# deprekate/PHANOTATE

Hardware: AMD Instinct MI355X
Metric: Mbp/s annotated (whole node) on 50 kb synthetic phage contigs (higher is better)
Workload: dtype u8 bases / fp64 scores / int64 edge weights / int128 distances; 1 GPU; batch of 1000 synthetic 50000 bp phage contigs on one GPU, resident in HBM (BASELINE config 4); contigs_total=1000, contigs_rank0=1000, contig_length=50000

## Files before the change

### include/phx.h

```cpp
#ifndef PHX_H
#define PHX_H

#include <stddef.h>
#include <stdint.h>

#ifdef __cplusplus
extern "C" {
#endif

#define PHX_VERSION 410
#define PHX_MAX_CODONS 16

#define PHX_OK 0
#define PHX_E_ARG (-1)
#define PHX_E_NODEVICE (-10)
#define PHX_E_HIP (-11)
#define PHX_E_NOMEM (-12)
#define PHX_E_STATE (-13)
#define PHX_E_PARAM (-14)
#define PHX_E_IO (-15)

#define PHX_S_OK 0
#define PHX_S_BADLETTER (-2)
#define PHX_S_TOOSHORT (-3)
// ... 157 lines not shown
    int32_t called;
    int32_t bypass;
} phx_gene_drop;
int phx_drop_margins_flat(phx_ctx *ctx, phx_gene_drop *rec, int64_t cap, int64_t *offsets , int32_t *status , int64_t *total);
int phx_drop_ms(phx_ctx *ctx, float *ms );
int phx_drop_stats(phx_ctx *ctx, int64_t *out );

int phx_dump_text(phx_ctx *ctx, int32_t contig, char **text, int64_t *text_len);

int phx_solve(phx_ctx *ctx, int32_t V, int32_t E, const int32_t *src, const int32_t *dst, const uint64_t *w_limbs,
              int32_t n_limbs, int32_t source, int32_t target, int32_t *path_out, int32_t cap, int32_t *n_path,
              uint64_t *dist_limbs);

#define PHX_N_STAGES 14
int phx_set_profiling(phx_ctx *ctx, int on);
int phx_set_profiling_stages(phx_ctx *ctx, uint32_t stage_mask);
int phx_get_stage_ms(phx_ctx *ctx, float *ms , int32_t *launches , int reset);
const char *phx_stage_name(int k);
int64_t phx_plan_timeouts(phx_ctx *ctx);
int64_t phx_front_runs(phx_ctx *ctx);
int64_t phx_seg_runs(phx_ctx *ctx);
int64_t phx_seg_fallbacks(phx_ctx *ctx);
int phx_seg_stats(phx_ctx *ctx, int32_t i, int32_t *out, int32_t cap_records);
int phx_batch_sizes(phx_ctx *ctx, int64_t *L, int64_t *n_orf, int64_t *n_node, int64_t *n_edge);

int phx_synth_contig(uint64_t seed, int64_t L, char *out);
int phx_dec_eval(const char *op, const char *a, const char *b, int prec, char *out, int cap);
int phx_dd_eval(const char *op, double ah, double al, double bh, double bl, double *rh, double *rl);
int phx_dd_shortest(double x, uint64_t *digits, int32_t *exp10);

typedef struct phx_fasta phx_fasta;
int phx_fasta_read(const char *path, phx_fasta **out);
int32_t phx_fasta_count(const phx_fasta *f);
int phx_fasta_record(const phx_fasta *f, int32_t i, const char **name, const char **seq, int64_t *len);
int phx_fasta_arrays(const phx_fasta *f, const char **names, const char **seqs, int64_t *lens);
void phx_fasta_free(phx_fasta *f);
int phx_format_tabular(int32_t n, const char *const *names, const phx_gene *genes, const int64_t *offsets, const int32_t *status, char **text, int64_t *text_len);
int phx_format_margins(int32_t n, const char *const *names, const phx_orf_margin *rec, const int64_t *offsets, const int32_t *status, char **text, int64_t *text_len);
int phx_format_drops(int32_t n, const char *const *names, const phx_gene_drop *rec, const int64_t *offsets, const int32_t *status, char **text, int64_t *text_len);
void phx_free_text(char *text);

#ifdef __cplusplus
}
#endif
#endif
```

### phanotate_amd/_lib.py

```python
import ctypes as C
import os

import numpy as np

HERE = os.path.dirname(os.path.abspath(__file__))
SO = os.path.join(HERE, "libphx.so")
MAXC = 16
N_STAGES = 14


class Params(C.Structure):
    _fields_ = [
        ("minlen", C.c_int32),
        ("n_start", C.c_int32),
        ("start", (C.c_char * 4) * MAXC),
        ("start_w", C.c_double * MAXC),
        ("n_stop", C.c_int32),
        ("stop", (C.c_char * 4) * MAXC),
        ("start_w_text", (C.c_char * 32) * MAXC),
    ]


class Gene(C.Structure):
    _fields_ = [("left", C.c_int32), ("right", C.c_int32), ("strand", C.c_int32), ("frame", C.c_int32), ("score", C.c_double)]
# ... 100 lines not shown
        "phx_tap_nodes": (C.c_int, [vp, i32, vp]),
        "phx_tap_edges": (C.c_int, [vp, i32, vp]),
        "phx_tap_path": (C.c_int, [vp, i32, vp, i32, P(i32), vp, i32]),
        "phx_tap_dist": (C.c_int, [vp, i32, vp, i64]),
        "phx_tap_dist_target": (C.c_int, [vp, i32, vp, i64]),
        "phx_margins_flat": (C.c_int, [vp, vp, i64, vp, vp, P(i64)]),
        "phx_margins_ms": (C.c_int, [vp, P(C.c_float)]),
        "phx_format_margins": (C.c_int, [i32, vp, vp, vp, vp, P(vp), P(i64)]),
        "phx_drop_margins_flat": (C.c_int, [vp, vp, i64, vp, vp, P(i64)]),
        "phx_drop_ms": (C.c_int, [vp, P(C.c_float)]),
        "phx_drop_stats": (C.c_int, [vp, P(i64)]),
        "phx_format_drops": (C.c_int, [i32, vp, vp, vp, vp, P(vp), P(i64)]),
        "phx_solve": (C.c_int, [vp, i32, i32, vp, vp, vp, i32, i32, i32, vp, i32, P(i32), vp]),
        "phx_set_profiling": (C.c_int, [vp, C.c_int]),
        "phx_set_profiling_stages": (C.c_int, [vp, C.c_uint32]),
        "phx_get_stage_ms": (C.c_int, [vp, P(C.c_float), P(i32), C.c_int]),
        "phx_stage_name": (C.c_char_p, [C.c_int]),
        "phx_batch_sizes": (C.c_int, [vp, P(i64), P(i64), P(i64), P(i64)]),
        "phx_plan_timeouts": (C.c_int64, [vp]),
        "phx_front_runs": (C.c_int64, [vp]),
        "phx_seg_runs": (C.c_int64, [vp]),
        "phx_seg_fallbacks": (C.c_int64, [vp]),
        "phx_seg_stats": (C.c_int, [vp, C.c_int32, C.c_void_p, C.c_int32]),
        "phx_synth_contig": (C.c_int, [C.c_uint64, i64, C.c_char_p]),
        "phx_fasta_read": (C.c_int, [C.c_char_p, P(vp)]),
        "phx_fasta_count": (i32, [vp]),
        "phx_fasta_record": (C.c_int, [vp, i32, P(vp), P(vp), P(i64)]),
        "phx_fasta_arrays": (C.c_int, [vp, vp, vp, vp]),
        "phx_fasta_free": (None, [vp]),
        "phx_format_tabular": (C.c_int, [i32, vp, vp, vp, vp, P(vp), P(i64)]),
        "phx_free_text": (None, [vp]),
    }
    for name, (res, args) in sig.items():
        f = getattr(L, name)
        f.restype = res
        f.argtypes = args
    assert GENE_DT.itemsize == C.sizeof(Gene)
    assert MARGIN_DT.itemsize == 40
    assert DROP_DT.itemsize == 40
    _lib = L
    return L


EXPORTS = ["phx_version", "phx_device_count", "phx_strerror", "phx_last_error", "phx_default_params", "phx_params_from_flags", "phx_set_exact", "phx_pool_create", "phx_pool_destroy", "phx_pool_last_error", "phx_pool_annotate", "phx_dump_text", "phx_dec_eval", "phx_dd_eval", "phx_dd_shortest", "phx_create", "phx_create_ex", "phx_destroy",
           "phx_annotate", "phx_free_results", "phx_upload", "phx_attach", "phx_set_trnas", "phx_run", "phx_run_async", "phx_wait", "phx_download", "phx_download_flat", "phx_certified", "phx_tap_globals",
           "phx_tap_positions", "phx_tap_orfs", "phx_tap_nodes", "phx_tap_edges", "phx_tap_path", "phx_tap_dist", "phx_solve", "phx_set_profiling", "phx_set_profiling_stages",
           "phx_get_stage_ms", "phx_stage_name", "phx_batch_sizes", "phx_plan_timeouts", "phx_front_runs", "phx_seg_runs", "phx_seg_fallbacks", "phx_seg_stats", "phx_synth_contig", "phx_fasta_read", "phx_fasta_count",
           "phx_fasta_record", "phx_fasta_arrays", "phx_fasta_free", "phx_format_tabular", "phx_free_text",
           "phx_margins_flat", "phx_tap_dist_target", "phx_margins_ms", "phx_format_margins",
           "phx_drop_margins_flat", "phx_drop_ms", "phx_drop_stats", "phx_format_drops"]
```

### phanotate_amd/api.py

```python
import ctypes as C

import numpy as np

from . import _lib
from ._lib import PhxError


def make_params(start_codons="atg:0.85,gtg:0.10,ttg:0.05", stop_codons="tag,tga,taa", minlen=90):
    p = _lib.Params()
    rc = _lib.lib().phx_params_from_flags(start_codons.encode(), stop_codons.encode(), int(minlen), C.byref(p))
    if rc:
        raise ValueError("start / stop codons %r / %r, minlen %r: libphx takes codon:weight pairs and codons of exactly 3 letters out of acgt, "
                         "at most %d of each, minlen >= 6 (%s)" % (start_codons, stop_codons, minlen, _lib.MAXC, _lib.lib().phx_strerror(rc).decode()))
    p.start_codons_text = start_codons
    return p


def synth_contig(seed, L=50000):
    buf = C.create_string_buffer(int(L))
    rc = _lib.lib().phx_synth_contig(int(seed), int(L), buf)
    if rc:
        raise PhxError(rc, "phx_synth_contig")
    return buf.raw

# ... 352 lines not shown

    def stage_ms(self, reset=True):
        ms = (C.c_float * _lib.N_STAGES)()
        nl = (C.c_int32 * _lib.N_STAGES)()
        self._chk(self.L.phx_get_stage_ms(self.h, ms, nl, 1 if reset else 0), "phx_get_stage_ms")
        return {self.L.phx_stage_name(k).decode(): (float(ms[k]), int(nl[k])) for k in range(_lib.N_STAGES)}

    def front_runs(self):
        return int(self.L.phx_front_runs(self.h))

    def seg_runs(self):
        return int(self.L.phx_seg_runs(self.h))

    def seg_fallbacks(self):
        return int(self.L.phx_seg_fallbacks(self.h))

    def seg_stats(self, i):
        import numpy as np

        out = np.zeros((64, 8), np.int32)
        n = self.L.phx_seg_stats(self.h, int(i), out.ctypes.data_as(C.c_void_p), 64)
        return out[:n]

    def plan_timeouts(self):
        return int(self.L.phx_plan_timeouts(self.h))

    def batch_sizes(self):
        v = [C.c_int64() for _ in range(4)]
        self._chk(self.L.phx_batch_sizes(self.h, *[C.byref(x) for x in v]), "phx_batch_sizes")
        return dict(L=v[0].value, n_orf=v[1].value, n_node=v[2].value, n_edge=v[3].value)
```

### phanotate_amd/csrc/phx_api.cpp

```cpp
#include <hip/hip_runtime.h>

#include <algorithm>
#include <atomic>
#include <cmath>
#include <condition_variable>
#include <functional>
#include <mutex>
#include <cstdio>
#include <cstdlib>
#include <cstring>
#include <memory>
#include <map>
#include <string>
#include <thread>
#include <vector>

#include "phx_internal.h"
extern "C" {
#include "phx_dec.h"
}

namespace {

thread_local std::string g_create_error;
// ... 139 lines not shown
    DTotals *h_tot = nullptr;
    bool have_plan = false;
    int last_mask = 0;
    int last_vmax = 0;
    int64_t last_lds[4] = {0, 0, 0, 0};
    int64_t max_len = 0;
    bool graphs_enabled = true, graph_valid = false, tiles_dirty = true;
    hipGraph_t graph = nullptr;
    hipGraphExec_t graph_exec = nullptr;
    int graph_flags = -1;
    void *h_stage = nullptr;
    size_t h_stage_cap = 0;
    DGene *h_genes = nullptr; size_t h_genes_cap = 0;
    bool prof = false;
    uint32_t prof_mask = 0xffffffffu;
    int n_simd = 1024;
    bool force_global_sssp = false;
    bool no_wave = false, always_sync = false;
    bool no_fuse = false;
    bool duo = true;
    int front_spins = 8000;
    bool side_score = true;
    int orf_stream = 1;
    bool orf_rows = true;
    bool eager_cert = true;
    bool pend_cert = false;
    bool pend_front = false;
    bool front_off = false;
    int64_t front_runs = 0;
    bool seg_on = true;
    bool seg_off = false;
    bool seg_never = false;
    bool pend_seg = false;
    int pend_seg_k = 0;
    bool seg_clean = false;
    int seg_max_n = 32;
    int seg_margin_bp = 6000;
    int64_t seg_runs = 0, seg_aborts = 0, seg_fallbacks = 0;
    DevBuf b_swin, b_swrole, b_sdist, b_segw;
    int64_t plan_timeouts = 0;
    bool plan_stream_off = false;
    DevBuf b_mo, b_md, b_mw, b_mdt, b_mrec, b_mstat;
    bool margins_done = false;
    phx_orf_margin *h_mrec = nullptr; size_t h_mrec_cap = 0;
    std::vector<int32_t> mstat;
    std::vector<DGrp> mgrp;
// ... 389 lines not shown
    if (!out || (flags & ~(PHX_CREATE_USE_STREAM | PHX_CREATE_NO_GRAPH | PHX_CREATE_SIZE_EVERY_RUN | PHX_CREATE_SOLVER_GLOBAL | PHX_CREATE_SOLVER_NO_WAVE | PHX_CREATE_NO_CERTIFY | PHX_CREATE_CERT_TIGHT | PHX_CREATE_CERT_WIDE | PHX_CREATE_POISON | PHX_CREATE_ONE_STREAM | PHX_CREATE_NO_EXACT | PHX_CREATE_NO_FUSE | PHX_CREATE_NO_DUO | PHX_CREATE_NO_SEG)) || (stream && !(flags & PHX_CREATE_USE_STREAM))) return PHX_E_ARG;
    *out = nullptr;
    int rc = check_params(params);
    if (rc) return rc;
    int ndev = 0;
    hipError_t e = hipGetDeviceCount(&ndev);
    if (e != hipSuccess || ndev <= 0 || device < 0 || device >= ndev) {
        g_create_error = e != hipSuccess ? hipGetErrorString(e) : "device index out of range";
        return PHX_E_NODEVICE;
    }
    phx_ctx *c = new phx_ctx();
    c->device = device;
    c->params = *params;
    c->force_global_sssp = (flags & PHX_CREATE_SOLVER_GLOBAL) != 0;
    c->no_wave = (flags & PHX_CREATE_SOLVER_NO_WAVE) != 0;
    c->graphs_enabled = (flags & PHX_CREATE_NO_GRAPH) == 0;
    c->always_sync = (flags & PHX_CREATE_SIZE_EVERY_RUN) != 0;
    c->certify = (flags & PHX_CREATE_NO_CERTIFY) == 0;
    c->exact = (flags & PHX_CREATE_NO_EXACT) == 0;
    c->no_fuse = (flags & PHX_CREATE_NO_FUSE) != 0;
    { const char *e = getenv("PHX_FRONT_SPINS"); if (e && *e) c->front_spins = atoi(e); }
    { const char *e = getenv("PHX_NO_EAGER_CERT"); c->eager_cert = !(e && e[0] == '1'); }
    { const char *e = getenv("PHX_NO_ORF_ROWS"); c->orf_rows = !(e && e[0] == '1'); }
    { const char *e = getenv("PHX_ORF_STREAM"); if (e && *e) { const int v = atoi(e); if (v >= -1 && v <= 3) c->orf_stream = v; } }
    { const char *e = getenv("PHX_NO_SIDE_SCORE"); c->side_score = !(e && e[0] == '1'); }
    { const char *e = getenv("PHX_NO_DUO"); c->duo = !(flags & PHX_CREATE_NO_DUO) && !(e && e[0] == '1'); }
    { const char *e = getenv("PHX_NO_SEG"); c->seg_on = !(flags & PHX_CREATE_NO_SEG) && !(e && e[0] == '1'); }
    { const char *e = getenv("PHX_SEG_MAX_N"); if (e && atoi(e) >= 0) c->seg_max_n = atoi(e); }
    { const char *e = getenv("PHX_SEG_MARGIN_BP"); if (e && atoi(e) > 0) c->seg_margin_bp = atoi(e); }
    c->cert_wide = (flags & PHX_CREATE_CERT_WIDE) != 0;
    c->poison = (flags & PHX_CREATE_POISON) != 0;
    c->cert_scale = (flags & PHX_CREATE_CERT_TIGHT) ? 68719476736.0 : 1.0;
    auto fail = [&](int code) { g_create_error = c->err; phx_destroy(c); return code; };
    if (hipSetDevice(device) != hipSuccess) { c->err = "hipSetDevice failed"; return fail(PHX_E_NODEVICE); }
    { int cus = 0; if (hipDeviceGetAttribute(&cus, hipDeviceAttributeMultiprocessorCount, device) == hipSuccess && cus > 0) c->n_simd = 4 * cus; }
    if (flags & PHX_CREATE_USE_STREAM) {
        c->stream = (hipStream_t)stream; c->own_stream = false;
        if (!stream) c->graphs_enabled = false;
    } else {
        if (hipStreamCreateWithFlags(&c->stream, hipStreamNonBlocking) != hipSuccess) { c->err = "hipStreamCreate failed"; return fail(PHX_E_HIP); }
        c->own_stream = true;
    }
    for (int a = 0; a < 4; a++) {
        if (flags & PHX_CREATE_ONE_STREAM) { c->aux[a] = c->stream; c->one_stream = true; }
        else if (hipStreamCreateWithFlags(&c->aux[a], hipStreamNonBlocking) != hipSuccess) { c->err = "hipStreamCreate failed"; return fail(PHX_E_HIP); }
        if (hipEventCreateWithFlags(&c->ev_join[a], hipEventDisableTiming) != hipSuccess) { c->err = "hipEventCreate failed"; return fail(PHX_E_HIP); }
// ... 392 lines not shown
        if ((rc = ensure(c, c->b_dist, ((size_t)ht->node + 8) * 8 * (size_t)c->n_limbs))) return rc;
        if (c->certify && (rc = ensure(c, c->b_csig, ((size_t)ht->node + 8) * 16 * (size_t)c->n_limbs))) return rc;
        if ((rc = ensure_seg(c))) return rc;
        mask = ht->class_mask;
        if (mask & 4) mask |= 8;
        for (int k = 0; k < 4; k++) lds[k] = ht->lds_need[k];
    }
    }
    fill_batch(c, &b);
    int stream_k = -1;
    if (c->n <= std::min(PHX_PLAN_STREAM_MAX, c->n_simd * 3 / 4) && !c->plan_stream_off && !b.sord && !c->one_stream && c->aux[3]) {
        if ((mask >> 2) & 1) stream_k = 0;
        else for (int k = 1; k <= 2; k++) if (((mask >> (4 * k + 2)) & 1) && !(mask & 0xffff & ~(15 << (4 * k)))) stream_k = k;
    }
    b.seg = (((mask >> 2) & 1) && seg_ready(c, b.caps)) ? seg_cap(c) : 0;
    c->pend_seg = b.seg != 0; c->pend_seg_k = b.seg;
    if (b.seg && stream_k == 0) stream_k = -1;
    b.seg_nofb = (b.seg && c->seg_clean && !learn) ? 1 : 0;
    b.seg_stream = (b.seg && !head_done && !learn && c->n <= 4 && !c->plan_stream_off && !c->one_stream && c->aux[3]) ? 1 : 0;
    const bool stream_plan = stream_k >= 0;
    b.duo = (c->duo && c->n <= c->n_simd) ? 1 : 0;
    b.plan_stream = stream_k < 0 ? 0 : (2 << stream_k);
    b.defer_overlap = c->max_len < (1 << 21) ? 1 : 0;
    auto launch_plan = [&]() -> int {
        HIPCHK(c, hipEventRecord(c->ev_fork_plan, s));
        HIPCHK(c, hipStreamWaitEvent(c->aux[3], c->ev_fork_plan, 0));
        {
            StageTimer t(c, ST_WAVE_PLAN, c->aux[3]);
            phxk_wave_plan(&b, ((mask >> 6) & 1) | (((mask >> 10) & 1) << 1), c->aux[3]);
            if (b.sord) phxk_sssp_order(&b, c->aux[3]);
        }
        HIPCHK(c, hipEventRecord(c->ev_join[3], c->aux[3]));
        return PHX_OK;
    };
    if ((rc = launch_plan())) return rc;
    b.orf_rows = (!fuse && c->orf_rows && c->n >= 600 && !c->one_stream && c->aux[2]) ? 1 : 0;
    const bool orf_side = b.orf_rows && c->orf_stream >= 0;
    if (orf_side) {
        hipStream_t so = c->aux[c->orf_stream];
        HIPCHK(c, hipEventRecord(c->ev_fork_orf, s));
        HIPCHK(c, hipStreamWaitEvent(so, c->ev_fork_orf, 0));
        phxk_edges_orf(&b, so);
        HIPCHK(c, hipEventRecord(c->ev_join_orf, so));
    }
    if (!fuse) { StageTimer t(c, ST_EDGE_FILL); if (b.orf_rows && !orf_side) phxk_edges_orf(&b, s); phxk_edges_fill(&b, s); if (orf_side) HIPCHK(c, hipStreamWaitEvent(s, c->ev_join_orf, 0)); }
    {
        StageTimer t(c, ST_SSSP);
        if (stream_plan) phxk_sssp(&b, 2 << stream_k, 2, (size_t)lds[stream_k], s);
        if (b.seg_stream) phxk_sssp(&b, 2, 2, (size_t)lds[0], s);
        HIPCHK(c, hipStreamWaitEvent(s, c->ev_join[3], 0));
        const int nl_of[4] = {2, 4, 8, 17};
        int nlaunch = 0, nclass = 0;
        bool used[3] = {false, false, false};
        for (int k = 0; k < 4; k++) nclass += ((mask >> (4 * k)) & 15) ? 1 : 0;
        bool early = false;
        auto early_k = [&](int k) { return ((mask >> (4 * k + 2)) & 1) && ((mask >> (4 * k + 1)) & 1) && (((mask >> (16 + k)) | (mask >> (20 + k))) & 1); };
        for (int k = 0; k < 4; k++) early = early || early_k(k);
        early = early && c->aux[2];
        const bool roomy_side = ((mask >> 3) & 1) && c->aux[2] && !c->one_stream;
        if ((nclass > 1 || early || roomy_side) && c->aux[0]) HIPCHK(c, hipEventRecord(c->ev_fork, s));
        if (early || roomy_side) {
            HIPCHK(c, hipStreamWaitEvent(c->aux[2], c->ev_fork, 0));
            used[2] = true;
            if (roomy_side) phxk_sssp(&b, 2, 3, 0, c->aux[2]);
            if (early)
                for (int k = 3; k >= 0; k--)
                    if (early_k(k)) phxk_sssp(&b, nl_of[k], 1, (size_t)lds[k], c->aux[2]);
            HIPCHK(c, hipEventRecord(c->ev_join[2], c->aux[2]));
        }
        for (int k = 3; k >= 0; k--) {
            if (!((mask >> (4 * k)) & 15)) continue;
            hipStream_t st = s;
            if (nlaunch > 0 && c->aux[0]) {
// ... 1395 lines not shown
}
const char *phx_stage_name(int k) { return k >= 0 && k < PHX_N_STAGES ? kStageName[k] : ""; }
int64_t phx_seg_runs(phx_ctx *c) {
    if (!c) return 0;
    if (c->in_flight && phx_wait(c)) return 0;
    return c->seg_runs;
}
int64_t phx_seg_fallbacks(phx_ctx *c) {
    if (!c) return 0;
    if (c->in_flight && phx_wait(c)) return 0;
    return c->seg_fallbacks;
}
int phx_seg_stats(phx_ctx *c, int32_t i, int32_t *out, int32_t cap_records) {
    if (!c || !out) return 0;
    if (c->in_flight && phx_wait(c)) return 0;
    if (i < 0 || i >= c->n || !c->ran || !c->pend_seg || !c->b_segw.p) return 0;
    if (hipSetDevice(c->device) != hipSuccess || hipStreamSynchronize(c->stream) != hipSuccess) return 0;
    const int K = c->pend_seg_k;
    const int n = std::min(K, (int)cap_records);
    if (n <= 0) return 0;
    if (hipMemcpy(out, (const int32_t *)c->b_segw.p + (size_t)i * (size_t)K * 8, (size_t)n * 32, hipMemcpyDeviceToHost) != hipSuccess) return 0;
    return n;
}
int64_t phx_front_runs(phx_ctx *c) {
    if (!c) return PHX_E_ARG;
    if (c->in_flight) { const int rs = phx_wait(c); if (rs) return rs; }
    return c->front_off ? -c->front_runs - 1 : c->front_runs;
}

int64_t phx_plan_timeouts(phx_ctx *c) {
    if (!c) return PHX_E_ARG;
    if (c->in_flight) { const int rs = phx_wait(c); if (rs) return rs; }
    return c->plan_timeouts;
}

int phx_batch_sizes(phx_ctx *c, int64_t *L, int64_t *n_orf, int64_t *n_node, int64_t *n_edge) {
    if (!c) return PHX_E_ARG;
    if (c->in_flight) { const int rs = phx_wait(c); if (rs) return rs; }
    if (L) *L = c->totalL;
    if (n_orf) *n_orf = c->tot_orf;
    if (n_node) *n_node = c->tot_node;
    if (n_edge) *n_edge = c->tot_edge;
    return PHX_OK;
}

}
// ... 1 lines not shown
```

### phanotate_amd/csrc/phx_internal.h

```cpp
#pragma once
#include <hip/hip_runtime.h>
#include <stdint.h>

#include "../../include/phx.h"

#define PHX_TILE 1536
#define PHX_CTG_THREADS 256
#define PHX_N_CODON_BITMAPS 12
#define PHX_PLANE_GCF 4
#define PHX_PLANE_GCR 7
#define PHX_PLANE_ATG 10
#define PHX_PRE_G 2
#define PHX_BITMAP_WORDS_PER_NW (PHX_N_CODON_BITMAPS * 3)

#define CLS_NONE 0
#define CLS_FS 1
#define CLS_RS 2
#define CLS_FT 3
#define CLS_RT 4

#define ESRC_F_GAP 0x20000000u
#define ESRC_GAP_NODES (1 << 19)
#define ESRC_IS_GAP(x) (((x) >> 29) & 1u)
#define ESRC_GAP_CODE(x) (((x) >> 19) & 1023u)
// ... 284 lines not shown
extern "C" {
#endif
void phx_pack_planes(const char *in, int64_t n, uint32_t *out, int64_t nrec);
void phxk_features(const DBatch *b, uint32_t v_begin, uint32_t v_end, void *stream);
void phxk_features_tap(const DBatch *b, int contig, uint32_t v_begin, uint32_t v_end, uint32_t *tapbuf, void *stream);
void phxk_pack_planes(const DBatch *b, const void *letters, void *stream);
void phxk_orf_count(const DBatch *b, void *stream);
void phxk_orf_emit(const DBatch *b, void *stream);
void phxk_bit_prefix(const DBatch *b, void *stream);
void phxk_orf_stats(const DBatch *b, void *stream);
void phxk_score(const DBatch *b, void *stream);
void phxk_nodes(const DBatch *b, void *stream);
void phxk_node_attr(const DBatch *b, void *stream);
void phxk_edges_count(const DBatch *b, void *stream);
void phxk_layout1(const DBatch *b, void *stream);
void phxk_layout2(const DBatch *b, void *stream);
void phxk_edges_fill(const DBatch *b, void *stream);
void phxk_edges_orf(const DBatch *b, void *stream);
void phxk_edges_expand(const DBatch *b, int n_limbs, int mode, void *stream);
void phxk_edges_tap(const DBatch *b, void *stream);
void phxk_sssp_order(const DBatch *b, void *stream);
size_t phxk_sssp_lds_bytes(int V, int n_limbs);
void phxk_wave_plan(const DBatch *b, int wide_too, void *stream);
int phxk_sssp_wave_ok(int n_limbs);
void phxk_sssp(const DBatch *b, int n_limbs, int mode, size_t lds_bytes, void *stream);
void phxk_inorder(const DBatch *b, int nl_mask, void *stream);
void phxk_refine(const DBatch *b, void *stream);
void phxk_certify(const DBatch *b, int nl_mask, int vmax, void *stream);
void phxk_gene_pack(const DBatch *b, void *stream);
void phxk_reset(const DBatch *b, const void *meta0, unsigned long long nbits_words, unsigned long long tbits_words, void *stream);
int phxk_front_blocks_y(const DBatch *b);
void phxk_front(const DBatch *b, void *stream);
void phxk_seg_merge(const DBatch *b, int vmax, void *stream);
int phxk_seg_kmax(void);
void phxk_seg_fallback(const DBatch *b, void *stream);
void phxk_results(const DBatch *b, void *stream);
void phxk_margins_transpose(const DBatch *b, const DMarg *g, void *stream);
void phxk_sssp_rev(const DBatch *b, const DMarg *g, int nl_mask, void *stream);
void phxk_margins(const DBatch *b, const DMarg *g, int nl_mask, void *stream);
void phxk_drop_trees(const DBatch *b, const DMarg *g, const DDrop *q, int nl_mask, void *stream);
void phxk_drop_cand(const DBatch *b, const DMarg *g, const DDrop *q, int nl_mask, void *stream);
void phxk_drop_fix(const DBatch *b, const DMarg *g, const DDrop *q, int nl_mask, void *stream);
#ifdef __cplusplus
}
#endif
```

### phanotate_amd/csrc/phx_kernels.hip

```cpp
#include <hip/hip_runtime.h>
#include <type_traits>

#include "phx_internal.h"

#define NT PHX_CTG_THREADS

__device__ __forceinline__ uint32_t wave_incl_scan(uint32_t v) {
    const int lane = threadIdx.x & 63;
#pragma unroll
    for (int d = 1; d < 64; d <<= 1) {
        uint32_t t = __shfl_up(v, d);
        if (lane >= d) v += t;
    }
    return v;
}
__device__ __forceinline__ uint32_t wave_incl_max(uint32_t v) {
    const int lane = threadIdx.x & 63;
#pragma unroll
    for (int d = 1; d < 64; d <<= 1) {
        uint32_t t = __shfl_up(v, d);
        if (lane >= d) v = v > t ? v : t;
    }
    return v;
}
// ... 80 lines not shown
}

__device__ __forceinline__ long long edge_wenc(uint32_t sw, const long long *ew, uint32_t e, const long long *gt) { return ESRC_IS_GAP(sw) ? gt[ESRC_GAP_CODE(sw)] : ew[e]; }
__device__ __forceinline__ const long long *gtab_of(const DBatch &b, const DMeta *meta) { return b.gtab ? b.gtab + (size_t)(meta - b.meta) * GT_N : nullptr; }

__device__ __forceinline__ double contig_pstop(uint32_t gc, int L) {
    double fa = (double)((uint32_t)L - gc), fg = (double)gc;
    double d = (double)((int64_t)L * 2);
    double Pa = fa / d, Pt = fa / d, Pg = fg / d;
    return Pt * Pa * Pa + Pt * Pg * Pa + Pt * Pa * Pg;
}
__device__ __forceinline__ int max_idx(int a, int b, int c) { return a > b ? (a > c ? 1 : 3) : (b > c ? 2 : 3); }
__device__ __forceinline__ int min_idx(int a, int b, int c) { return a > b ? (b > c ? 3 : 2) : (a > c ? 3 : 1); }

#include "phx_features.inc"
#include "phx_orf.inc"
#include "phx_graph.inc"
#include "phx_sssp.inc"
#include "phx_layout.inc"
#include "phx_front.inc"
#include "phx_sssp_seg.inc"
#include "phx_sssp_wave.inc"
#include "phx_sssp_duo.inc"
#include "phx_inorder.inc"
#include "phx_refine.inc"
#include "phx_certify.inc"
#include "phx_margins.inc"
#include "phx_drop.inc"

template <int NL>
static void launch_certify(const DBatch *b, int vcap, hipStream_t s) {
    const size_t lds = (size_t)vcap * 12 + 16;
    if (lds > 48 * 1024) (void)hipFuncSetAttribute((const void *)k_certify<NL>, hipFuncAttributeMaxDynamicSharedMemorySize, (int)lds);
    hipLaunchKernelGGL(k_certify<NL>, dim3(b->n_contig), dim3(CERT_T), lds, s, *b, vcap);
    hipLaunchKernelGGL(k_certify_wide<NL>, dim3(b->n_contig), dim3(CERT_T), 0, s, *b);
}
extern "C" {
void phxk_features(const DBatch *b, uint32_t v_begin, uint32_t v_end, void *stream) {
    if (v_end <= v_begin) return;
    const unsigned g = (v_end - 1) / FEAT_SPAN - v_begin / FEAT_SPAN + 1;
    if (b->defcod) hipLaunchKernelGGL((k_features<false, true>), dim3(g), dim3(64), 0, (hipStream_t)stream, *b, v_begin, v_end, (uint32_t *)nullptr, -1);
    else hipLaunchKernelGGL((k_features<false, false>), dim3(g), dim3(64), 0, (hipStream_t)stream, *b, v_begin, v_end, (uint32_t *)nullptr, -1);
}
void phxk_features_tap(const DBatch *b, int contig, uint32_t v_begin, uint32_t v_end, uint32_t *tapbuf, void *stream) {
    if (v_end <= v_begin) return;
    const unsigned g = (v_end - 1) / FEAT_SPAN - v_begin / FEAT_SPAN + 1;
// ... 165 lines not shown
    DP_LAUNCH(k_dp_rec, nl_mask);
}
size_t phxk_sssp_lds_bytes(int V, int nl) { return sssp_lds_bytes(V, nl); }
void phxk_layout1(const DBatch *b, void *stream) {
    if (b->n_contig <= LAYOUT_T) { hipLaunchKernelGGL(k_layout1, dim3(1), dim3(LAYOUT_T), 0, (hipStream_t)stream, *b); return; }
    const unsigned g = (unsigned)((b->n_contig + LMB_T - 1) / LMB_T);
    hipLaunchKernelGGL(k_layout1_a, dim3(g), dim3(LMB_T), 0, (hipStream_t)stream, *b);
    hipLaunchKernelGGL(k_layout1_b, dim3(g), dim3(LMB_T), 0, (hipStream_t)stream, *b);
}
void phxk_layout2(const DBatch *b, void *stream) {
    if (b->n_contig <= LAYOUT_T) { hipLaunchKernelGGL(k_layout2, dim3(1), dim3(LAYOUT_T), 0, (hipStream_t)stream, *b); return; }
    const unsigned g = (unsigned)((b->n_contig + LMB_T - 1) / LMB_T);
    hipLaunchKernelGGL(k_layout2_a, dim3(g), dim3(LMB_T), 0, (hipStream_t)stream, *b);
    hipLaunchKernelGGL(k_layout2_b, dim3(g), dim3(LMB_T), 0, (hipStream_t)stream, *b);
}

void phxk_sssp_order(const DBatch *b, void *stream) { hipLaunchKernelGGL(k_sssp_order, dim3(1), dim3(LMB_T), 0, (hipStream_t)stream, *b); }

int phxk_sssp_wave_ok(int nl) { return nl == 2 || nl == 4 || nl == 8; }
void phxk_wave_plan(const DBatch *b, int wide_too, void *stream) {
    if (b->seg) hipLaunchKernelGGL((k_wave_plan<2, 0, true>), dim3(b->n_contig * b->seg), dim3(64), 0, (hipStream_t)stream, *b);
    else hipLaunchKernelGGL((k_wave_plan<2, 0>), dim3(b->n_contig), dim3(64), 0, (hipStream_t)stream, *b);
    hipLaunchKernelGGL((k_wave_plan<2, 1>), dim3(b->n_contig), dim3(64), 0, (hipStream_t)stream, *b);
    if (wide_too & 1) hipLaunchKernelGGL((k_wave_plan<4, 1>), dim3(b->n_contig), dim3(64), 0, (hipStream_t)stream, *b);
    if (wide_too & 2) hipLaunchKernelGGL((k_wave_plan<8, 1>), dim3(b->n_contig), dim3(64), 0, (hipStream_t)stream, *b);
}

void phxk_sssp(const DBatch *b, int nl, int mode, size_t lds_bytes, void *stream) {
    dim3 g(b->n_contig), t(NT);
    hipStream_t s = (hipStream_t)stream;
    if ((mode == 2 || mode == 3) && !(mode == 2 && nl == 2 && b->duo) && b->gtab && b->gap_code) phxk_edges_expand(b, nl, mode, stream);
    if (mode == 2 || mode == 3) {
        if (nl == 2 && mode == 2 && b->duo) {
            dim3 t2(128);
            if (b->seg && b->seg_stream) hipLaunchKernelGGL((k_sssp_duo<0, true, true>), dim3(b->n_contig * b->seg), t2, 0, s, *b);
            else if (b->seg) hipLaunchKernelGGL((k_sssp_duo<0, false, true>), dim3(b->n_contig * b->seg), t2, 0, s, *b);
            else if (b->plan_stream == 2) hipLaunchKernelGGL((k_sssp_duo<0, true>), g, t2, 0, s, *b);
            else hipLaunchKernelGGL((k_sssp_duo<0, false>), g, t2, 0, s, *b);
        } else if (nl == 2 && mode == 2) {
            const size_t lb = wv_lds_bytes<2, 0>();
            (void)hipFuncSetAttribute((const void *)k_sssp_wave<2, 0>, hipFuncAttributeMaxDynamicSharedMemorySize, (int)lb);
            if (b->plan_stream == 2) {
                (void)hipFuncSetAttribute((const void *)k_sssp_wave<2, 0, true>, hipFuncAttributeMaxDynamicSharedMemorySize, (int)lb);
                hipLaunchKernelGGL((k_sssp_wave<2, 0, true>), g, dim3(64), lb, s, *b);
            } else
            hipLaunchKernelGGL((k_sssp_wave<2, 0>), g, dim3(64), lb, s, *b);
// ... 51 lines not shown
```

Measured before the change: 32610 Mbp/s.

## Parallelize SSSP wave planning across a 512-thread block on the main stream

Adds a new wave-plan kernel that builds the 2-limb window schedule with a block-wide prefix scan over node degrees, a per-thread binary search for window extents, a serial window chain on one thread, and per-wave role setup. It replaces the 64-thread sequential k_wave_plan launches. By default this kernel runs inline on the main stream, and the side-stream fork/join is skipped unless wide plans or sssp ordering are needed. It also adds a debug tap to read back windows. The risks are mismatched window decisions compared with the old planner and heavier use of LDS per block.

```diff
diff --git a/include/phx.h b/include/phx.h
--- a/include/phx.h
+++ b/include/phx.h
@@ -203,6 +203,7 @@
 int64_t phx_seg_runs(phx_ctx *ctx);
 int64_t phx_seg_fallbacks(phx_ctx *ctx);
 int phx_seg_stats(phx_ctx *ctx, int32_t i, int32_t *out, int32_t cap_records);
+int phx_tap_windows(phx_ctx *ctx, int32_t i, int32_t *meta4, void *win, void *roles, int32_t cap);
 int phx_batch_sizes(phx_ctx *ctx, int64_t *L, int64_t *n_orf, int64_t *n_node, int64_t *n_edge);
 
 int phx_synth_contig(uint64_t seed, int64_t L, char *out);
diff --git a/phanotate_amd/_lib.py b/phanotate_amd/_lib.py
--- a/phanotate_amd/_lib.py
+++ b/phanotate_amd/_lib.py
@@ -146,6 +146,7 @@
         "phx_seg_runs": (C.c_int64, [vp]),
         "phx_seg_fallbacks": (C.c_int64, [vp]),
         "phx_seg_stats": (C.c_int, [vp, C.c_int32, C.c_void_p, C.c_int32]),
+        "phx_tap_windows": (C.c_int, [vp, C.c_int32, P(i32), vp, vp, C.c_int32]),
         "phx_synth_contig": (C.c_int, [C.c_uint64, i64, C.c_char_p]),
         "phx_fasta_read": (C.c_int, [C.c_char_p, P(vp)]),
         "phx_fasta_count": (i32, [vp]),
@@ -169,7 +170,7 @@
 EXPORTS = ["phx_version", "phx_device_count", "phx_strerror", "phx_last_error", "phx_default_params", "phx_params_from_flags", "phx_set_exact", "phx_pool_create", "phx_pool_destroy", "phx_pool_last_error", "phx_pool_annotate", "phx_dump_text", "phx_dec_eval", "phx_dd_eval", "phx_dd_shortest", "phx_create", "phx_create_ex", "phx_destroy",
            "phx_annotate", "phx_free_results", "phx_upload", "phx_attach", "phx_set_trnas", "phx_run", "phx_run_async", "phx_wait", "phx_download", "phx_download_flat", "phx_certified", "phx_tap_globals",
            "phx_tap_positions", "phx_tap_orfs", "phx_tap_nodes", "phx_tap_edges", "phx_tap_path", "phx_tap_dist", "phx_solve", "phx_set_profiling", "phx_set_profiling_stages",
-           "phx_get_stage_ms", "phx_stage_name", "phx_batch_sizes", "phx_plan_timeouts", "phx_front_runs", "phx_seg_runs", "phx_seg_fallbacks", "phx_seg_stats", "phx_synth_contig", "phx_fasta_read", "phx_fasta_count",
+           "phx_get_stage_ms", "phx_stage_name", "phx_batch_sizes", "phx_plan_timeouts", "phx_front_runs", "phx_seg_runs", "phx_seg_fallbacks", "phx_seg_stats", "phx_tap_windows", "phx_synth_contig", "phx_fasta_read", "phx_fasta_count",
            "phx_fasta_record", "phx_fasta_arrays", "phx_fasta_free", "phx_format_tabular", "phx_free_text",
            "phx_margins_flat", "phx_tap_dist_target", "phx_margins_ms", "phx_format_margins",
            "phx_drop_margins_flat", "phx_drop_ms", "phx_drop_stats", "phx_format_drops"]
diff --git a/phanotate_amd/api.py b/phanotate_amd/api.py
--- a/phanotate_amd/api.py
+++ b/phanotate_amd/api.py
@@ -398,6 +398,17 @@
         n = self.L.phx_seg_stats(self.h, int(i), out.ctypes.data_as(C.c_void_p), 64)
         return out[:n]
 
+    def tap_windows(self, i, cap=4096):
+        import numpy as np
+
+        meta = (C.c_int32 * 4)()
+        win = np.zeros((cap, 8), np.int32)
+        roles = np.zeros((cap, 128, 2), np.uint32)
+        n = self.L.phx_tap_windows(self.h, int(i), meta, win.ctypes.data_as(C.c_void_p), roles.ctypes.data_as(C.c_void_p), int(cap))
+        if n < 0:
+            self._chk(n, "phx_tap_windows")
+        return list(meta), win[:n], roles[:n]
+
     def plan_timeouts(self):
         return int(self.L.phx_plan_timeouts(self.h))
 
diff --git a/phanotate_amd/csrc/phx_api.cpp b/phanotate_amd/csrc/phx_api.cpp
--- a/phanotate_amd/csrc/phx_api.cpp
+++ b/phanotate_amd/csrc/phx_api.cpp
@@ -185,6 +185,7 @@
     int front_spins = 8000;
     bool side_score = true;
     int orf_stream = 1;
+    bool side_plan = false;
     bool orf_rows = true;
     bool eager_cert = true;
     bool pend_cert = false;
@@ -620,6 +621,7 @@
     { const char *e = getenv("PHX_FRONT_SPINS"); if (e && *e) c->front_spins = atoi(e); }
     { const char *e = getenv("PHX_NO_EAGER_CERT"); c->eager_cert = !(e && e[0] == '1'); }
     { const char *e = getenv("PHX_NO_ORF_ROWS"); c->orf_rows = !(e && e[0] == '1'); }
+    { const char *e = getenv("PHX_SIDE_PLAN"); c->side_plan = e && e[0] == '1'; }
     { const char *e = getenv("PHX_ORF_STREAM"); if (e && *e) { const int v = atoi(e); if (v >= -1 && v <= 3) c->orf_stream = v; } }
     { const char *e = getenv("PHX_NO_SIDE_SCORE"); c->side_score = !(e && e[0] == '1'); }
     { const char *e = getenv("PHX_NO_DUO"); c->duo = !(flags & PHX_CREATE_NO_DUO) && !(e && e[0] == '1'); }
@@ -1058,12 +1060,18 @@
     b.duo = (c->duo && c->n <= c->n_simd) ? 1 : 0;
     b.plan_stream = stream_k < 0 ? 0 : (2 << stream_k);
     b.defer_overlap = c->max_len < (1 << 21) ? 1 : 0;
+    const int wide_too = ((mask >> 6) & 1) | (((mask >> 10) & 1) << 1);
+    const bool par_plan = !stream_plan && !b.seg && !c->side_plan;
+    const bool side_plan = !par_plan || wide_too || b.sord;
     auto launch_plan = [&]() -> int {
+        if (par_plan) { StageTimer t(c, ST_EDGE_FILL); phxk_wave_plan_par(&b, s); }
+        if (!side_plan) return PHX_OK;
         HIPCHK(c, hipEventRecord(c->ev_fork_plan, s));
         HIPCHK(c, hipStreamWaitEvent(c->aux[3], c->ev_fork_plan, 0));
         {
             StageTimer t(c, ST_WAVE_PLAN, c->aux[3]);
-            phxk_wave_plan(&b, ((mask >> 6) & 1) | (((mask >> 10) & 1) << 1), c->aux[3]);
+            if (par_plan) phxk_wave_plan_wide(&b, wide_too, c->aux[3]);
+            else phxk_wave_plan(&b, wide_too, c->aux[3]);
             if (b.sord) phxk_sssp_order(&b, c->aux[3]);
         }
         HIPCHK(c, hipEventRecord(c->ev_join[3], c->aux[3]));
@@ -1084,7 +1092,7 @@
         StageTimer t(c, ST_SSSP);
         if (stream_plan) phxk_sssp(&b, 2 << stream_k, 2, (size_t)lds[stream_k], s);
         if (b.seg_stream) phxk_sssp(&b, 2, 2, (size_t)lds[0], s);
-        HIPCHK(c, hipStreamWaitEvent(s, c->ev_join[3], 0));
+        if (side_plan) HIPCHK(c, hipStreamWaitEvent(s, c->ev_join[3], 0));
         const int nl_of[4] = {2, 4, 8, 17};
         int nlaunch = 0, nclass = 0;
         bool used[3] = {false, false, false};
@@ -2526,6 +2534,19 @@
     if (hipMemcpy(out, (const int32_t *)c->b_segw.p + (size_t)i * (size_t)K * 8, (size_t)n * 32, hipMemcpyDeviceToHost) != hipSuccess) return 0;
     return n;
 }
+int phx_tap_windows(phx_ctx *c, int32_t i, int32_t *meta4, void *win, void *roles, int32_t cap) {
+    if (!c || !meta4) return PHX_E_ARG;
+    if (c->in_flight) { const int rs = phx_wait(c); if (rs) return rs; }
+    if (i < 0 || i >= c->n || !c->ran) return PHX_E_ARG;
+    if (hipSetDevice(c->device) != hipSuccess || hipStreamSynchronize(c->stream) != hipSuccess) return PHX_E_HIP;
+    DMeta m;
+    if (hipMemcpy(&m, (const DMeta *)c->b_meta.p + i, sizeof(DMeta), hipMemcpyDeviceToHost) != hipSuccess) return PHX_E_HIP;
+    meta4[0] = m.n_win; meta4[1] = m.sssp_mode; meta4[2] = m.sssp_why; meta4[3] = m.sssp_nl;
+    const int n = std::max(0, std::min(m.n_win, cap));
+    if (n && win && hipMemcpy(win, (const DWin *)c->b_win.p + m.win_off, sizeof(DWin) * (size_t)n, hipMemcpyDeviceToHost) != hipSuccess) return PHX_E_HIP;
+    if (n && roles && hipMemcpy(roles, (const uint2 *)c->b_wrole.p + (size_t)m.win_off * WIN_ROLES, sizeof(uint2) * WIN_ROLES * (size_t)n, hipMemcpyDeviceToHost) != hipSuccess) return PHX_E_HIP;
+    return n;
+}
 int64_t phx_front_runs(phx_ctx *c) {
     if (!c) return PHX_E_ARG;
     if (c->in_flight) { const int rs = phx_wait(c); if (rs) return rs; }
diff --git a/phanotate_amd/csrc/phx_internal.h b/phanotate_amd/csrc/phx_internal.h
--- a/phanotate_amd/csrc/phx_internal.h
+++ b/phanotate_amd/csrc/phx_internal.h
@@ -330,6 +330,8 @@
 void phxk_sssp_order(const DBatch *b, void *stream);
 size_t phxk_sssp_lds_bytes(int V, int n_limbs);
 void phxk_wave_plan(const DBatch *b, int wide_too, void *stream);
+void phxk_wave_plan_par(const DBatch *b, void *stream);
+void phxk_wave_plan_wide(const DBatch *b, int wide_too, void *stream);
 int phxk_sssp_wave_ok(int n_limbs);
 void phxk_sssp(const DBatch *b, int n_limbs, int mode, size_t lds_bytes, void *stream);
 void phxk_inorder(const DBatch *b, int nl_mask, void *stream);
diff --git a/phanotate_amd/csrc/phx_kernels.hip b/phanotate_amd/csrc/phx_kernels.hip
--- a/phanotate_amd/csrc/phx_kernels.hip
+++ b/phanotate_amd/csrc/phx_kernels.hip
@@ -126,6 +126,7 @@
 #include "phx_sssp_seg.inc"
 #include "phx_sssp_wave.inc"
 #include "phx_sssp_duo.inc"
+#include "phx_plan_par.inc"
 #include "phx_inorder.inc"
 #include "phx_refine.inc"
 #include "phx_certify.inc"
@@ -337,6 +338,13 @@
     if (b->seg) hipLaunchKernelGGL((k_wave_plan<2, 0, true>), dim3(b->n_contig * b->seg), dim3(64), 0, (hipStream_t)stream, *b);
     else hipLaunchKernelGGL((k_wave_plan<2, 0>), dim3(b->n_contig), dim3(64), 0, (hipStream_t)stream, *b);
     hipLaunchKernelGGL((k_wave_plan<2, 1>), dim3(b->n_contig), dim3(64), 0, (hipStream_t)stream, *b);
+    if (wide_too & 1) hipLaunchKernelGGL((k_wave_plan<4, 1>), dim3(b->n_contig), dim3(64), 0, (hipStream_t)stream, *b);
+    if (wide_too & 2) hipLaunchKernelGGL((k_wave_plan<8, 1>), dim3(b->n_contig), dim3(64), 0, (hipStream_t)stream, *b);
+}
+void phxk_wave_plan_par(const DBatch *b, void *stream) {
+    hipLaunchKernelGGL(k_wave_plan_par, dim3(b->n_contig), dim3(PP_THREADS), 0, (hipStream_t)stream, *b);
+}
+void phxk_wave_plan_wide(const DBatch *b, int wide_too, void *stream) {
     if (wide_too & 1) hipLaunchKernelGGL((k_wave_plan<4, 1>), dim3(b->n_contig), dim3(64), 0, (hipStream_t)stream, *b);
     if (wide_too & 2) hipLaunchKernelGGL((k_wave_plan<8, 1>), dim3(b->n_contig), dim3(64), 0, (hipStream_t)stream, *b);
 }
diff --git a/phanotate_amd/csrc/phx_plan_par.inc b/phanotate_amd/csrc/phx_plan_par.inc
--- /dev/null
+++ b/phanotate_amd/csrc/phx_plan_par.inc
@@ -0,0 +1,230 @@
+#define PP_T 1024
+#define PP_EXT (PP_T + 132)
+#define PP_THREADS 512
+#define PP_WAVES (PP_THREADS / 64)
+#define PP_WMAX 128
+#define PP_CHUNK ((PP_EXT + PP_THREADS - 1) / PP_THREADS)
+static_assert(PP_CHUNK * PP_THREADS >= PP_EXT, "scan chunks");
+static_assert(PP_EXT * 65 < (1 << 17) && PP_EXT < (1 << 15), "prefix fields");
+
+__global__ __launch_bounds__(PP_THREADS) void k_wave_plan_par(DBatch b) {
+    constexpr int CA = WvNum<2>::CA, CB = WvNum<2>::CB;
+    __shared__ uint4 s_nd[PP_EXT];
+    __shared__ uint16_t s_nx[PP_T];
+    __shared__ int4 s_win[PP_WMAX];
+    __shared__ uint32_t s_wt[2 * PP_WAVES];
+    __shared__ uint8_t s_lists[PP_WAVES][2 * 128];
+    __shared__ uint4 s_recs[PP_WAVES][64];
+    __shared__ uint8_t s_heads[PP_WAVES][64];
+    __shared__ int s_st[8];
+
+    const int ci = (int)blockIdx.x;
+    DMeta *meta = &b.meta[ci];
+    const int V = meta->n_node;
+    const int mode0 = meta->sssp_mode;
+    if (b.tot->overflow || meta->status < 0 || V <= 2 || meta->sssp_nl != 2 || (mode0 != 2 && mode0 != 3)) return;
+    const int tid = threadIdx.x, lane = tid & 63, wid = tid >> 6;
+    const uint64_t below = lane ? (~0ull >> (64 - lane)) : 0ull;
+    const int SRC = V - 2;
+    const uint32_t *in_off = b.in_off + meta->node_off + ci;
+    const DNode *nd = b.node + meta->node_off;
+    const uint32_t *mreach = b.mreach + 4 * (size_t)meta->node_off;
+    const bool mr_partial = (meta->dense & 2) != 0;
+    DWin *win = b.win + meta->win_off;
+    uint2 *wrole = b.wrole + (size_t)meta->win_off * WIN_ROLES;
+    const int win_cap = V / 16 + 7;
+    uint8_t *s_listA = s_lists[wid], *s_listB = s_lists[wid] + 128;
+    uint4 *s_rec = s_recs[wid];
+    uint8_t *s_head = s_heads[wid];
+
+    for (int cfg = mode0 == 2 ? 0 : 1;; cfg++) {
+        const uint32_t ECAP = cfg ? WvDims<2, 1>::ECAP : WvDims<2, 0>::ECAP;
+        const int OV = cfg ? WvDims<2, 1>::OV : WvDims<2, 0>::OV;
+        if (tid == 0) { s_st[0] = 0; s_st[1] = -1; s_st[2] = 0; s_st[3] = 0; s_st[4] = 0; s_st[5] = 0; }
+        __syncthreads();
+        int t0 = 0;
+        for (;;) {
+            for (int i = tid; i < PP_EXT; i += PP_THREADS) {
+                const int c = t0 + i;
+                const uint32_t x = in_off[c < V ? c : V];
+                const int y = c < SRC ? nd[c].pos : WV_POS_INF;
+                uint32_t u1 = 0, u2 = 0;
+                if (c < V) {
+                    const int deg = (int)(in_off[c + 1] - x), inf = nd[c].info;
+                    const bool k = (NTYPE(inf) == 1 && NFRAME(inf) > 0) || (NTYPE(inf) == 0 && NFRAME(inf) < 0);
+                    int q = k ? (deg > CA ? (deg + CA - 1) / CA : 1) : (deg > CB ? (deg + CB - 1) / CB : 1);
+                    q = q > 65 ? 65 : q;
+                    if (k) u1 = (uint32_t)q | (1u << 17); else u2 = (uint32_t)q;
+                }
+                s_nd[i] = make_uint4(x, (uint32_t)y, u1, u2);
+            }
+            __syncthreads();
+            {
+                const int i0 = tid * PP_CHUNK;
+                uint32_t a1 = 0, a2 = 0;
+                for (int r = 0; r < PP_CHUNK; r++) if (i0 + r < PP_EXT) { a1 += s_nd[i0 + r].z; a2 += s_nd[i0 + r].w; }
+                const uint32_t c1 = wv_scan(a1), c2 = wv_scan(a2);
+                if (lane == 63) { s_wt[wid] = c1; s_wt[PP_WAVES + wid] = c2; }
+                __syncthreads();
+                uint32_t r1 = c1 - a1, r2 = c2 - a2;
+                for (int w = 0; w < wid; w++) { r1 += s_wt[w]; r2 += s_wt[PP_WAVES + w]; }
+                for (int r = 0; r < PP_CHUNK; r++)
+                    if (i0 + r < PP_EXT) {
+                        const uint4 e = s_nd[i0 + r];
+                        s_nd[i0 + r] = make_uint4(e.x, e.y, (r1 & 0xffffu) | (r2 << 16), r1 >> 17);
+                        r1 += e.z; r2 += e.w;
+                    }
+            }
+            __syncthreads();
+            for (int i = tid; i < PP_T; i += PP_THREADS) {
+                const int s = t0 + i;
+                uint16_t nx = 0;
+                if (s < V) {
+                    const uint4 e0 = s_nd[i];
+                    const int hi = V - s < 128 ? V - s : 128;
+                    auto ok = [&](int j, bool budget) -> bool {
+                        const uint4 e = s_nd[i + j + 1];
+                        if (e.x - e0.x > ECAP) return false;
+                        if (budget && j > 0 && (((e.z - e0.z) & 0xffffu) > 64u || (((e.z >> 16) - (e0.z >> 16)) & 0xffffu) > 64u)) return false;
+                        if (j >= 64) { const int nc = (int)(e.w - e0.w); if (nc > 64 || j + 1 - nc > 64) return false; }
+                        return true;
+                    };
+                    auto nmax_of = [&](bool budget) {
+                        int n = 0;
+                        for (int st = 128; st; st >>= 1) if (n + st <= hi && ok(n + st - 1, budget)) n += st;
+                        return n;
+                    };
+                    auto amax_of = [&](int nmax) {
+                        if (s + nmax >= V) return nmax;
+                        const int lim = (int)s_nd[i + nmax].y;
+                        int n = 0;
+                        for (int st = 128; st; st >>= 1) if (n + st <= nmax && (int)s_nd[i + n + st - 1].y + 500 <= lim) n += st;
+                        return n;
+                    };
+                    int nmax = nmax_of(true), amax = amax_of(nmax);
+                    if (amax < 8) { nmax = nmax_of(false); amax = amax_of(nmax); }
+                    const int a = amax < WV_ADV ? amax : WV_ADV;
+                    if (a > 0) {
+                        const int pl = (int)s_nd[i + a - 1].y + 500;
+                        int n = a;
+                        for (int st = 128; st; st >>= 1) if (n + st <= nmax && (int)s_nd[i + n + st - 1].y < pl) n += st;
+                        nx = (uint16_t)(a | (n << 8));
+                    }
+                }
+                s_nx[i] = nx;
+            }
+            __syncthreads();
+            if (tid == 0) {
+                int s = s_st[0], prev = s_st[1], k = s_st[2], state = 0, nw = 0;
+                if (k == 0 && s_nx[0] == 0) state = 2;
+                while (!state) {
+                    if (k >= win_cap) { state = 2; break; }
+                    const int i = s - t0;
+                    const int nx = s_nx[i], a = nx & 255, va = s + a;
+                    const bool last = va >= V;
+                    if (!last) {
+                        if (va - t0 >= PP_T) break;
+                        if (s_nx[va - t0] == 0) { state = 2; break; }
+                    }
+                    if (nw == PP_WMAX) break;
+                    const int pl = (int)s_nd[i + a - 1].y + 500;
+                    s_win[nw++] = make_int4(s, va, s + (nx >> 8), pl);
+                    k++;
+                    if (last) { state = 1; break; }
+                    prev = pl; s = va;
+                }
+                s_st[6] = s_st[1]; s_st[7] = s_st[2];
+                s_st[0] = s; s_st[1] = prev; s_st[2] = k; s_st[3] = state; s_st[4] = nw;
+            }
+            __syncthreads();
+            const int nw = s_st[4], kbase = s_st[7], prev0 = s_st[6];
+            for (int m = wid; m < nw; m += PP_WAVES) {
+                const int4 wr = s_win[m];
+                const int v0 = wr.x, base = v0 - t0, nwin = wr.z - v0;
+                const int prev_lim = m ? s_win[m - 1].w : prev0;
+                const uint32_t e0 = s_nd[base].x;
+                const bool in1 = lane < nwin, in2 = 64 + lane < nwin;
+                const bool k1 = in1 && s_nd[base + lane + 1].w != s_nd[base + lane].w;
+                const bool k2 = in2 && s_nd[base + 64 + lane + 1].w != s_nd[base + 64 + lane].w;
+                const uint64_t mc1 = __ballot(k1), mo1 = __ballot(in1 && !k1), mc2 = __ballot(k2), mo2 = __ballot(in2 && !k2);
+                const int nc = __popcll(mc1) + __popcll(mc2), no = __popcll(mo1) + __popcll(mo2);
+                wv_sync();
+                if (in1) { if (k1) s_listA[__popcll(mc1 & below)] = (uint8_t)lane; else s_listB[__popcll(mo1 & below)] = (uint8_t)lane; }
+                if (in2) { if (k2) s_listA[__popcll(mc1) + __popcll(mc2 & below)] = (uint8_t)(64 + lane); else s_listB[__popcll(mo1) + __popcll(mo2 & below)] = (uint8_t)(64 + lane); }
+                wv_sync();
+                int n_spill = 0;
+                auto setup = [&](const uint8_t *list, int n, const int cap, const bool close, uint32_t &summary) -> uint2 {
+                    const bool own = lane < n;
+                    const int jn = own ? list[lane] : 0;
+                    const uint32_t o0 = own ? s_nd[base + jn].x : 0u, o1 = own ? s_nd[base + jn + 1].x : 0u;
+                    const int deg = (int)(o1 - o0), i0 = (int)(o0 - e0);
+                    const int want = own ? (deg > cap ? (deg + cap - 1) / cap : 1) : 0;
+                    const int extra = want - (own ? 1 : 0);
+                    const int ex_incl = (int)wv_scan((uint32_t)extra);
+                    int got = (64 - n) - (ex_incl - extra);
+                    got = got < 0 ? 0 : (got > extra ? extra : got);
+                    const int items = (own ? 1 : 0) + got;
+                    const int it_incl = (int)wv_scan((uint32_t)items);
+                    const int off = it_incl - items;
+                    const int total = wv_last(it_incl);
+                    const int spill = own ? (deg - items * cap > 0 ? deg - items * cap : 0) : 0;
+                    const int sp_incl = (int)wv_scan((uint32_t)spill);
+                    const int sp_off = n_spill + sp_incl - spill;
+                    n_spill += wv_last(sp_incl);
+                    wv_sync();
+                    s_head[lane] = 0;
+                    wv_sync();
+                    if (own) {
+                        s_rec[lane] = make_uint4((uint32_t)jn | ((uint32_t)off << 8) | ((uint32_t)items << 16), (uint32_t)i0, (uint32_t)deg, (uint32_t)(sp_off & 0xffff) | ((uint32_t)spill << 16));
+                        s_head[off] = 1;
+                    }
+                    wv_sync();
+                    const uint64_t hm = __ballot(s_head[lane] != 0);
+                    const bool act = lane < total;
+                    const int ow = __popcll(hm & (below | (1ull << lane))) - 1;
+                    const uint4 rc = act ? s_rec[ow] : make_uint4(0, 0, 0, 0);
+                    const int o_j = (int)(rc.x & 255), ch = act ? lane - (int)((rc.x >> 8) & 255) : 0, o_items = (int)(rc.x >> 16);
+                    const int o_i0 = (int)rc.y, o_deg = (int)rc.z, o_sp = (int)(rc.w & 0xffff), o_spn = (int)(rc.w >> 16);
+                    const bool head = act && ch == 0;
+                    const int nfollow = head ? o_items - 1 : 0;
+                    int cnt = o_deg - ch * cap;
+                    cnt = !act ? 0 : (cnt > cap ? cap : (cnt < 0 ? 0 : cnt));
+                    const int apos = (head && close && v0 + o_j < SRC) ? (int)s_nd[base + o_j].y : WV_POS_INF;
+                    const bool watch = prev_lim >= 0 && apos < prev_lim && (mr_partial || mreach[v0 + o_j] < (uint32_t)v0);
+                    summary = (uint32_t)total | ((uint32_t)wv_max(cnt) << 8) | ((uint32_t)wv_max(nfollow) << 16);
+                    return wv_role_pack(act, o_j, ch, nfollow, cnt, watch, o_i0 + ch * cap, head ? o_sp : 0, head ? o_spn : 0);
+                };
+                uint32_t sumA = 0, sumB = 0;
+                const uint2 rA = setup(s_listA, nc, CA, true, sumA);
+                const uint2 rB = setup(s_listB, no, CB, false, sumB);
+                const int kg = kbase + m;
+                if (n_spill > OV) { if (lane == 0) atomicOr(&s_st[5], 1); continue; }
+                wrole[(size_t)kg * WIN_ROLES + lane] = rA;
+                wrole[(size_t)kg * WIN_ROLES + 64 + lane] = rB;
+                if (lane == 0) {
+                    DWin w;
+                    w.v0 = v0; w.va = wr.y; w.v1 = wr.z; w.e0 = e0; w.ne = s_nd[base + nwin].x - e0; w.pa = sumA; w.pb = sumB; w.sp = (uint32_t)n_spill;
+                    win[kg] = w;
+                }
+            }
+            __syncthreads();
+            const int state = s_st[3], spilled = s_st[5];
+            if (state || spilled) break;
+            t0 = s_st[0];
+            __syncthreads();
+        }
+        const int state = s_st[3], fail_code = s_st[5] ? 2 : (state == 2 ? 1 : 0), k = s_st[2];
+        __syncthreads();
+        if (!fail_code) { if (tid == 0) meta->n_win = k; return; }
+        if (cfg == 0) {
+            if (tid == 0) { meta->sssp_mode = 3; meta->n_win = 0; atomicOr(&b.tot->class_mask, 1 << 3); }
+            continue;
+        }
+        if (tid == 0) {
+            meta->sssp_mode = meta->sssp_fb;
+            meta->sssp_why = fail_code; meta->n_win = 0;
+            atomicOr(&b.tot->class_mask, 1 << 20);
+        }
+        return;
+    }
+}
```

After: 31870 Mbp/s, median of 2. 0.977x the previous value.
